# Youncy-Hu/MAGE

Measured on AMD Instinct MI355X. Metric: generated frames/sec (64x64, 16-frame clips), higher is better.
Workload: dtype bf16

## Files before the change

mage_amd/csrc/gemm4.hip:

```cpp
#include <cstdio>
#include <cstdlib>
#include <utility>

#include "gemm_shared.h"
#include "gemm4_regs.h"
#include "attn_mfma.h"

namespace {

struct Gemm4Args {
    const void* A;
    const void* W;
    void* Y;
    const float* bias;
    const float* ln_stats;
    const float* ln_colsum;
    const void* residual;
    float* ln_part;
    void* y2;
    int M, N, K, lda, ldw, ldy, ldr, ldy2, y_dtype, a_off, y_off;
    int ntiles_n, ntiles;
    int stagger_groups, stagger_sleeps;
    alignas(16) int attn_axis;
    float attn_scale;
    int out_w, y_img_stride;
};

#ifndef MAGE4_ABL
#define MAGE4_ABL 0
#endif

#ifdef MAGE4_STAMP
__device__ unsigned long long g4_stamps[256 * 32 * 4 * 8];
#define G4_STAMP(it, p)                                                                                                   \
    do {                                                                                                                  \
        if (lane == 0 && (it) < 32 && blockIdx.x < 256) {                                                                 \
            g4_stamps[((blockIdx.x * 32 + (it)) * 4 + wave) * 8 + (p)] = __builtin_readcyclecounter();                    \
            if ((p) == 1) g4_stamps[((blockIdx.x * 32 + (it)) * 4 + wave) * 8 + 3] = __builtin_amdgcn_s_memrealtime();    \
            if ((p) == 0) g4_stamps[((blockIdx.x * 32 + (it)) * 4 + wave) * 8 + 4] = __builtin_amdgcn_s_memrealtime();    \
        }                                                                                                                 \
    } while (0)
#else
#define G4_STAMP(it, p)
#endif

constexpr int G4_STAGE = 65536, G4_WOFF = 32768, G4_RING = 2 * G4_STAGE, G4_LDS = G4_RING + 4 * 4096;

#ifdef MAGE4_MFMA32
template <int B, bool ZERO, bool CLOB>
__device__ __forceinline__ void g4_mfma32(const u32x4& w, const u32x4& x) {
    if constexpr (ZERO && CLOB) asm volatile("v_mfma_f32_32x32x16_bf16 a[%c2:%c3], %0, %1, 0" ::"v"(w), "v"(x), "i"(16 * B), "i"(16 * B + 15) : G4_ALL_ACC);
    else if constexpr (ZERO) asm volatile("v_mfma_f32_32x32x16_bf16 a[%c2:%c3], %0, %1, 0" ::"v"(w), "v"(x), "i"(16 * B), "i"(16 * B + 15));
    else if constexpr (CLOB) asm volatile("v_mfma_f32_32x32x16_bf16 a[%c2:%c3], %0, %1, a[%c2:%c3]" ::"v"(w), "v"(x), "i"(16 * B), "i"(16 * B + 15) : G4_ALL_ACC);
    else asm volatile("v_mfma_f32_32x32x16_bf16 a[%c2:%c3], %0, %1, a[%c2:%c3]" ::"v"(w), "v"(x), "i"(16 * B), "i"(16 * B + 15));
}
#endif
typedef unsigned g4_u32x2 __attribute__((ext_vector_type(2)));
template <bool HF>
__device__ __forceinline__ f32x4 g4_epi_qk(const u32x4& k, const u32x4& q) {
    f32x4 d;
    if constexpr (HF) asm volatile("s_nop 1\n\tv_mfma_f32_16x16x32_f16 %0, %1, %2, 0\n\ts_nop 15" : "=&v"(d) : "v"(k), "v"(q));
    else asm volatile("s_nop 1\n\tv_mfma_f32_16x16x32_bf16 %0, %1, %2, 0\n\ts_nop 15" : "=&v"(d) : "v"(k), "v"(q));
    return d;
}
#define G4_EPI_PV(OP)                                                                                                                               \
    asm volatile("s_nop 1\n\t" OP " %0, %2, %4, 0\n\t" OP " %1, %3, %4, 0\n\t" OP " %0, %2, %5, %0\n\t" OP " %1, %3, %5, %1\n\ts_nop 15"           \
                 : "=&v"(o0), "=&v"(o1)                                                                                                             \
                 : "v"(__builtin_bit_cast(g4_u32x2, vt0)), "v"(__builtin_bit_cast(g4_u32x2, vt1)), "v"(__builtin_bit_cast(g4_u32x2, phi)),          \
                   "v"(__builtin_bit_cast(g4_u32x2, plo)))
template <bool HF>
__device__ __forceinline__ void g4_epi_pv(const ashort4& vt0, const ashort4& vt1, const ashort4& phi, const ashort4& plo, f32x4& o0, f32x4& o1) {
    if constexpr (HF) G4_EPI_PV("v_mfma_f32_16x16x16_f16");
    else G4_EPI_PV("v_mfma_f32_16x16x16_bf16");
}

template <bool SWAP, int I, bool ZERO, bool CLOB, bool HF>
__device__ __forceinline__ void g4_mm(const u32x4& w, const u32x4& x) {
    if constexpr (SWAP) g4_mfma<I, ZERO, CLOB, HF>(x, w);
    else g4_mfma<I, ZERO, CLOB, HF>(w, x);
}
template <int ACT, int EK, int LN, bool RB, bool HF, bool QF, bool TX = false>
__device__ __forceinline__ void gemm4_body(const Gemm4Args& g) {
    static_assert(EK != EK_GENERAL, "lean epilogue kinds");
    static_assert(!TX || QF, "the temporal row map belongs to the fused attention entry");
    static_assert(!QF || (LN == LN_CONSUME && ACT == MAGE_ACT_NONE), "fused attention: the LayerNorm-consuming in_proj");
    static_assert(!HF || (LN != LN_DUAL && LN != LN_GELUBWD), "f16 form: the generation path's epilogues");
    typedef std::conditional_t<HF, f16_t, unsigned short> H16;
    extern __shared__ __attribute__((aligned(16))) char smem[];
    g4_claim_accumulators();
    const int tid = threadIdx.x;
    const int lane = tid & 63;
    const int wave = __builtin_amdgcn_readfirstlane(tid >> 6);
    const int nwg8 = gridDim.x >> 3;
    const int xcd = blockIdx.x & 7, li = blockIdx.x >> 3;
    const int q8 = g.ntiles >> 3, r8 = g.ntiles & 7;
    const int chunk0 = xcd < r8 ? xcd * (q8 + 1) : r8 * (q8 + 1) + (xcd - r8) * q8;
    const int chunk1 = chunk0 + q8 + (xcd < r8 ? 1 : 0);
    const int nk = g.K >> 6;
    int c_tile = chunk0 + li;
    if (c_tile >= chunk1) return;
    const int last_tile = c_tile + ((chunk1 - 1 - c_tile) / nwg8) * nwg8;

    const int lr = lane >> 3, lp = lane & 7;
    unsigned voffA[8], voffW[8];
    [[maybe_unused]] auto frame_row = [&](int R) {
        if constexpr (TX) return (R & 15) * g.out_w + (R >> 4);
        else return g.attn_axis == 1 ? ((R & 15) << 4) + (R >> 4) : R;
    };
    [[maybe_unused]] auto tile_row0 = [&](int tm_) {
        const int clip = tm_ / g.y_img_stride;
        return (long)clip * 16 * g.out_w + (tm_ - clip * g.y_img_stride) * 16;
    };
#pragma unroll
    for (int u = 0; u < 8; ++u) {
        const int r = u * 8 + lr;
        const int ch = lp ^ ((r >> 1) & 7);
        if constexpr (TX) voffA[u] = (unsigned)frame_row(wave * 64 + r) * (unsigned)(g.lda * 2) + (unsigned)(ch * 16 + 8192 - u * 1024);
        else voffA[u] = (unsigned)((QF ? frame_row(wave * 64 + r) : r) * g.lda * 2 + ch * 16 + 8192 - u * 1024);
        voffW[u] = (unsigned)(r * g.ldw * 2 + ch * 16 + 8192 - u * 1024);
    }
    auto a_base = [&](int tile) {
        if constexpr (TX) return (const char*)g.A + (tile_row0(tile / g.ntiles_n) + g.a_off) * g.lda * 2 - 4096;
        else return (const char*)g.A + ((long)((tile / g.ntiles_n) * 256 + (QF ? 0 : wave * 64)) + g.a_off) * g.lda * 2 - 4096;
    };
    auto w_base = [&](int tile) { return (const char*)g.W + (long)((tile % g.ntiles_n) * (QF ? 384 : 256) + wave * 64) * g.ldw * 2 - 4096; };
    [[maybe_unused]] auto w_base_v = [&](int tile) { return (const char*)g.W + (long)((tile % g.ntiles_n) * 384 + 256 + wave * 32) * g.ldw * 2 - 4096; };
    const char* a_src = a_base(c_tile);
    const char* w_src = w_base(c_tile);
    const char* a_next = a_src;
    const char* w_next = w_src;
    const unsigned lds0 = (unsigned)(uintptr_t)(__attribute__((address_space(3))) char*)smem + wave * 8192 + 4096;
    auto dma_m0 = [&](unsigned lds_group) __attribute__((always_inline)) {
        asm volatile("s_mov_b32 m0, %0\n\ts_nop 0" ::"s"(lds0 + lds_group) : "memory");
    };
    auto dma_m0w = [&](unsigned stage_off, bool half) __attribute__((always_inline)) { dma_m0(stage_off + G4_WOFF - (half ? wave * 4096 : 0)); };

    const int wm = wave >> 1, wn = wave & 1;
    const int l15 = lane & 15, grp = lane >> 4;
    const int rsw = (l15 >> 1) & 7;
    const int pc[2] = {((grp + 0) ^ rsw) * 16, ((grp + 4) ^ rsw) * 16};
    const int x_off = (wm * 128 + l15) * 128;
    const int w_off = G4_WOFF + (wn * 128 + l15) * 128;
    [[maybe_unused]] const int w_off_v = G4_WOFF + (wn * 64 + l15) * 128;
    u32x4 wf[2][8], xf[2][4];
    auto rd_w1 = [&](int buf, int stage, int t, int nt) __attribute__((always_inline)) {
        wf[buf][nt] = *(const u32x4*)(smem + stage * G4_STAGE + w_off + nt * 2048 + pc[t]);
    };
    [[maybe_unused]] auto rd_wv = [&](int buf, int stage, int t, int nt) __attribute__((always_inline)) {
        wf[buf][nt] = *(const u32x4*)(smem + stage * G4_STAGE + w_off_v + nt * 2048 + pc[t]);
    };
    auto rd_x1 = [&](int buf, int stage, int t, int mt) __attribute__((always_inline)) {
        xf[buf][mt & 3] = *(const u32x4*)(smem + stage * G4_STAGE + x_off + mt * 2048 + pc[t]);
    };

#ifdef MAGE4_MFMA32
    const int l31 = lane & 31, hi5 = lane >> 5;
    const int rsw32 = (l31 >> 1) & 7;
    const int x32_off = (wm * 128 + l31) * 128, w32_off = G4_WOFF + (wn * 128 + l31) * 128;
    u32x4 wq[2][4], xq[2][4];
    auto rd_w32 = [&](int buf, int stage, int ks, int nb) __attribute__((always_inline)) {
        wq[buf][nb] = *(const u32x4*)(smem + stage * G4_STAGE + w32_off + nb * 4096 + (((2 * ks + hi5) ^ rsw32) << 4));
    };
    auto rd_x32 = [&](int buf, int stage, int ks, int mb) __attribute__((always_inline)) {
        xq[buf][mb] = *(const u32x4*)(smem + stage * G4_STAGE + x32_off + mb * 4096 + (((2 * ks + hi5) ^ rsw32) << 4));
    };
#endif
    if (g.stagger_groups > 1) {
        for (int w = (li % g.stagger_groups) * g.stagger_sleeps; w > 0; --w) __builtin_amdgcn_s_sleep(16);
    }
    dma_m0(0);
    g4_for<8>([&](auto u_) { g4_dma<decltype(u_)::value>(voffA[decltype(u_)::value], a_src); });
    dma_m0(G4_WOFF);
    g4_for<8>([&](auto u_) { g4_dma<decltype(u_)::value>(voffW[decltype(u_)::value], w_src); });
    a_src += 128;
    w_src += 128;
    dma_m0(G4_STAGE);
    g4_for<8>([&](auto u_) { g4_dma<decltype(u_)::value>(voffA[decltype(u_)::value], a_src); });
    dma_m0(G4_STAGE + G4_WOFF);
    g4_for<8>([&](auto u_) { g4_dma<decltype(u_)::value>(voffW[decltype(u_)::value], w_src); });
    a_src += 128;
    w_src += 128;
    __builtin_amdgcn_s_waitcnt(0x0F70);
    ring_barrier();
#ifdef MAGE4_MFMA32
#pragma unroll
    for (int b = 0; b < 4; ++b) { rd_w32(0, 0, 0, b); rd_x32(0, 0, 0, b); }
#else
#pragma unroll
    for (int nt = 0; nt < 8; ++nt) rd_w1(0, 0, 0, nt);
#pragma unroll
    for (int m = 0; m < 4; ++m) rd_x1(0, 0, 0, m);
#endif

    [[maybe_unused]] int it = 0;
    for (; c_tile < chunk1; c_tile += nwg8, ++it) {
        G4_STAMP(it, 0);
        const int tm = c_tile / g.ntiles_n, tn = c_tile - tm * g.ntiles_n;
        MAGE_DASSERT(c_tile >= 0 && c_tile < g.ntiles && tm * 256 < g.M && tn * (QF ? 384 : 256) < g.N);
        [[maybe_unused]] float ln_mean[8], ln_rstd[8];
        [[maybe_unused]] long row0 = 0;
        if constexpr (TX) row0 = tile_row0(tm);
        auto tile = [&](auto PH_) __attribute__((always_inline)) {
            constexpr int PH = decltype(PH_)::value;
            constexpr bool HALF = PH == 2, KEEP = PH == 1;
            constexpr int NW = HALF ? 4 : 8;
            const int m0 = ((MAGE4_ABL & 32) ? (int)blockIdx.x : tm) * 256 + wm * 128;
            const int n0 = QF ? tn * 384 + (HALF ? 256 + wn * 64 : wn * 128) : ((MAGE4_ABL & 32) ? 0 : tn) * 256 + wn * 128;
            [[maybe_unused]] const int ny0 = HALF ? tn * 128 + wn * 64 : n0;
            if constexpr (KEEP) {
                if constexpr (TX) a_next = (const char*)g.A + (row0 + g.a_off) * g.lda * 2 - 4096;
                else a_next = a_base(c_tile);
                w_next = w_base_v(c_tile);
            } else {
                const int nt_tile = c_tile + nwg8 > last_tile ? last_tile : c_tile + nwg8;
                a_next = a_base(nt_tile);
                w_next = w_base(nt_tile);
            }
            auto rd_w = [&](int buf, int stage, int t, int nt) __attribute__((always_inline)) {
                if constexpr (HALF) rd_wv(buf, stage, t, nt);
                else rd_w1(buf, stage, t, nt);
            };
            f32x4 biasm[2][4];
            [[maybe_unused]] f32x4 lns[2][4];
            [[maybe_unused]] f32x4 pl[4][2];
            [[maybe_unused]] int ql15 = l15, qgrp = grp;
            if constexpr (QF) asm volatile("" : "+v"(ql15), "+v"(qgrp));
            auto slab = [&](auto S_, auto FIRST_, auto LAST_, int j) __attribute__((always_inline)) {
                constexpr int S = decltype(S_)::value;
                constexpr bool FIRST = decltype(FIRST_)::value, LAST = decltype(LAST_)::value;
                constexpr int ACC0 = HALF ? 32 : 0;
                constexpr bool WH_ = LAST ? KEEP : HALF;
                constexpr int WU = WH_ ? 4 : 8;
                g4_for<4 * NW>([&](auto i_) {
                    constexpr int i = decltype(i_)::value, m = i / NW, nt = i % NW;
                    g4_mm<PH == 2, ACC0 + ((nt >> 2) * 8 + m) * 4 + (nt & 3), FIRST, i == 0, HF>(wf[0][nt], xf[0][m]);
                    __builtin_amdgcn_sched_barrier(0);
                    if constexpr (!(MAGE4_ABL & 4) && i < 4) {
                        rd_x1(1, S, 0, 4 + i);
                        __builtin_amdgcn_sched_barrier(0);
                    }
                    if constexpr (!(MAGE4_ABL & 2) && !FIRST && i == 4) {
                        dma_m0w((S ^ 1) * G4_STAGE, WH_);
                        __builtin_amdgcn_sched_barrier(0);
                    }
                    if constexpr (!HALF) {
                        if constexpr (!(MAGE4_ABL & 2) && !FIRST && (i & 3) == 1 && i > 4 && (i >> 2) - 1 < WU) {
                            g4_dma<(i >> 2) - 1>(voffW[(i >> 2) - 1], w_src);
                            __builtin_amdgcn_sched_barrier(0);
                        }
                    } else {
                        if constexpr (!FIRST && i > 4 && i - 5 < WU) {
                            g4_dma<i - 5>(voffW[i - 5], w_src);
                            __builtin_amdgcn_sched_barrier(0);
                        }
                    }
                });
                if constexpr (!(MAGE4_ABL & 2) && !FIRST && !HALF && WU == 8) {
                    g4_dma<7>(voffW[7], w_src);
                    __builtin_amdgcn_sched_barrier(0);
                }
                if constexpr (!(MAGE4_ABL & 8) && !FIRST) w_src = (j == nk - 2) ? w_next : w_src + 128;
                g4_for<4 * NW>([&](auto i_) {
                    constexpr int i = decltype(i_)::value, m = i / NW, nt = i % NW;
                    g4_mm<PH == 2, ACC0 + ((nt >> 2) * 8 + 4 + m) * 4 + (nt & 3), FIRST, i == 0, HF>(wf[0][nt], xf[1][m]);
                    __builtin_amdgcn_sched_barrier(0);
                    if constexpr (!(MAGE4_ABL & 4) && i < 4 + NW) {
                        if constexpr (i < 4) rd_x1(0, S, 1, i);
                        else rd_w(1, S, 1, i - 4);
                        __builtin_amdgcn_sched_barrier(0);
                    }
                });
                if constexpr (LAST) {
#pragma unroll
                    for (int b = 0; b < 4; ++b) {
                        if constexpr (PH == 2) {
                            biasm[0][0][b] = g.bias[n0 + b * 16 + l15];
                            lns[0][0][b] = g.ln_colsum[n0 + b * 16 + l15];
                            continue;
                        }
                        const int n = n0 + b * 16 + grp * 4;
                        biasm[0][b] = *(const f32x4*)(g.bias + n);
                        if constexpr (LN == LN_CONSUME) lns[0][b] = *(const f32x4*)(g.ln_colsum + n);
                    }
                    if constexpr (LN == LN_CONSUME && !HALF) {
#pragma unroll
                        for (int a = 0; a < 8; ++a) {
                            long row;
                            if constexpr (TX) row = row0 + frame_row(wm * 128 + a * 16 + ql15);
                            else row = QF ? (long)tm * 256 + frame_row(wm * 128 + a * 16 + ql15) : (long)(m0 + a * 16 + l15);
                            const float2 st = *(const float2*)(g.ln_stats + 2 * row);
                            ln_mean[a] = st.x;
                            ln_rstd[a] = st.y;
                        }
                    }
                    __builtin_amdgcn_sched_barrier(0);
                }
                g4_for<4 * NW>([&](auto i_) {
                    constexpr int i = decltype(i_)::value, m = i / NW, nt = i % NW;
                    g4_mm<PH == 2, ACC0 + ((nt >> 2) * 8 + m) * 4 + (nt & 3), false, i == 0, HF>(wf[1][nt], xf[0][m]);
                    __builtin_amdgcn_sched_barrier(0);
                    if constexpr (!(MAGE4_ABL & 4) && i < 4) {
                        rd_x1(1, S, 1, 4 + i);
                        __builtin_amdgcn_sched_barrier(0);
                    }
                });
                if constexpr (MAGE4_ABL & 16) __builtin_amdgcn_s_waitcnt(0xC07F);
                else if constexpr (FIRST && QF) __builtin_amdgcn_s_waitcnt(PH == 1 ? 0x007C : 0x0070);
                else if constexpr (FIRST) __builtin_amdgcn_s_waitcnt(LN == LN_CONSUME ? 0x8074 : 0x8070);
                else __builtin_amdgcn_s_waitcnt(0x0070);
                ring_barrier();
                __builtin_amdgcn_sched_barrier(0);
                g4_for<4 * NW>([&](auto i_) {
                    constexpr int i = decltype(i_)::value, m = i / NW, nt = i % NW;
                    g4_mm<PH == 2, ACC0 + ((nt >> 2) * 8 + 4 + m) * 4 + (nt & 3), false, i == 0, HF>(wf[1][nt], xf[1][m]);
                    __builtin_amdgcn_sched_barrier(0);
                    if constexpr (!(MAGE4_ABL & 4) && i < 4 + NW && !LAST) {
                        if constexpr (i < 4) rd_x1(0, S ^ 1, 0, i);
                        else rd_w(0, S ^ 1, 0, i - 4);
                        __builtin_amdgcn_sched_barrier(0);
                    }
                    if constexpr (!(MAGE4_ABL & 2) && !LAST && !HALF) {
                        if constexpr (i == 2) dma_m0(S * G4_STAGE);
                        if constexpr ((i & 3) == 3) g4_dma<(i >> 2)>(voffA[i >> 2], a_src);
                        if constexpr (i == 2 || (i & 3) == 3) __builtin_amdgcn_sched_barrier(0);
                    }
                    if constexpr (!(MAGE4_ABL & 2) && LAST && !HALF) {
                        if constexpr (i == 0) dma_m0(S * G4_STAGE);
                        if constexpr (i == 16) dma_m0w(S * G4_STAGE, WH_);
                        if constexpr ((i & 1) == 1 && i < 16) g4_dma<(i >> 1)>(voffA[i >> 1], a_src);
                        if constexpr ((i & 1) == 1 && i > 16 && ((i - 16) >> 1) < WU) g4_dma<((i - 16) >> 1)>(voffW[(i - 16) >> 1], w_src);
                        if constexpr (i == 0 || i == 16 || (i & 1) == 1) __builtin_amdgcn_sched_barrier(0);
                    }
                    if constexpr (HALF && !LAST) {
                        if constexpr (i == 0) dma_m0(S * G4_STAGE);
                        if constexpr ((i & 1) == 1) g4_dma<(i >> 1)>(voffA[i >> 1], a_src);
                        if constexpr (i == 0 || (i & 1) == 1) __builtin_amdgcn_sched_barrier(0);
                    }
                    if constexpr (HALF && LAST) {
                        if constexpr (i == 0) dma_m0(S * G4_STAGE);
                        if constexpr (i == 8) dma_m0w(S * G4_STAGE, false);
                        if constexpr (i < 8) g4_dma<i>(voffA[i], a_src);
                        else g4_dma<i - 8>(voffW[i - 8], w_src);
                        __builtin_amdgcn_sched_barrier(0);
                    }
                });
                if constexpr (!(MAGE4_ABL & 8)) a_src = (j == nk - 3) ? a_next : a_src + 128;
                if constexpr (!(MAGE4_ABL & 8) && LAST) w_src += 128;
            };
#ifdef MAGE4_MFMA32
            auto slab32 = [&](auto S_, auto FIRST_, auto LAST_, int j) __attribute__((always_inline)) {
                constexpr int S = decltype(S_)::value;
                constexpr bool FIRST = decltype(FIRST_)::value, LAST = decltype(LAST_)::value;
                auto quarter = [&](auto Q_) __attribute__((always_inline)) {
                    constexpr int Q = decltype(Q_)::value, buf = Q & 1;
                    g4_for<16>([&](auto i_) {
                        constexpr int i = decltype(i_)::value, mb = i >> 2, nb = i & 3;
                        g4_mfma32<mb * 4 + nb, FIRST && Q == 0, i == 0>(wq[buf][nb], xq[buf][mb]);
                        __builtin_amdgcn_sched_barrier(0);
                        if constexpr (!(MAGE4_ABL & 4) && i < 8 && !(Q == 3 && LAST)) {
                            constexpr int st = Q == 3 ? (S ^ 1) : S, ks = (Q + 1) & 3;
                            if constexpr (i < 4) rd_x32(buf ^ 1, st, ks, i);
                            else rd_w32(buf ^ 1, st, ks, i - 4);
                            __builtin_amdgcn_sched_barrier(0);
                        }
                        if constexpr (Q == 0 && !(MAGE4_ABL & 2) && !FIRST) {
                            if constexpr (i == 4) dma_m0((S ^ 1) * G4_STAGE + G4_WOFF);
                            if constexpr (i >= 5 && i < 13) g4_dma<i - 5>(voffW[i - 5], w_src);
                            if constexpr (i >= 4 && i < 13) __builtin_amdgcn_sched_barrier(0);
                        }
                        if constexpr (Q == 3 && !(MAGE4_ABL & 2) && !LAST) {
                            if constexpr (i == 1) dma_m0(S * G4_STAGE);
                            if constexpr (i >= 2 && i < 10) g4_dma<i - 2>(voffA[i - 2], a_src);
                            if constexpr (i >= 1 && i < 10) __builtin_amdgcn_sched_barrier(0);
                        }
                    });
                };
                quarter(std::integral_constant<int, 0>{});
                if constexpr (!(MAGE4_ABL & 8) && !FIRST) w_src = (j == nk - 2) ? w_next : w_src + 128;
                quarter(std::integral_constant<int, 1>{});
                quarter(std::integral_constant<int, 2>{});
                if constexpr (FIRST) __builtin_amdgcn_s_waitcnt(0x8070);
                else __builtin_amdgcn_s_waitcnt(0x0070);
                ring_barrier();
                __builtin_amdgcn_sched_barrier(0);
                quarter(std::integral_constant<int, 3>{});
                if constexpr (LAST && !(MAGE4_ABL & 2)) {
                    dma_m0(S * G4_STAGE);
                    g4_for<8>([&](auto u_) { g4_dma<decltype(u_)::value>(voffA[decltype(u_)::value], a_src); });
                    dma_m0(S * G4_STAGE + G4_WOFF);
                    g4_for<8>([&](auto u_) { g4_dma<decltype(u_)::value>(voffW[decltype(u_)::value], w_src); });
                }
                if constexpr (!(MAGE4_ABL & 8)) a_src = (j == nk - 3) ? a_next : a_src + 128;
                if constexpr (!(MAGE4_ABL & 8) && LAST) w_src += 128;
            };
#define slab slab32
#endif
            typedef std::integral_constant<int, 0> S0;
            typedef std::integral_constant<int, 1> S1;
            slab(S0{}, std::true_type{}, std::false_type{}, 0);
            slab(S1{}, std::false_type{}, std::false_type{}, 1);
            for (int j = 2; j < nk - 2; j += 2) {
                slab(S0{}, std::false_type{}, std::false_type{}, j);
                slab(S1{}, std::false_type{}, std::false_type{}, j + 1);
            }
            slab(S0{}, std::false_type{}, std::false_type{}, nk - 2);
            slab(S1{}, std::false_type{}, std::true_type{}, nk - 1);
#ifdef MAGE4_MFMA32
#undef slab
#endif
            asm volatile("s_nop 15\n\ts_nop 7" ::: "memory");
            G4_STAMP(it, 1);
#if MAGE4_ABL & 1
            {
                f32x4 t = g4_acc_read<0>() + g4_acc_read<17>() + g4_acc_read<63>();
                if (t[0] + t[1] + t[2] + t[3] == 123456.789f) ((float*)g.Y)[0] = t[0] + biasm[0][0][0];
            }
#else
            char* win = smem + G4_RING + wave * 4096;
#pragma unroll
            for (int b = 0; b < (HALF ? 0 : 4); ++b) {
                if constexpr (PH == 2) {
                    biasm[1][0][b] = g.bias[n0 + 64 + b * 16 + l15];
                    lns[1][0][b] = g.ln_colsum[n0 + 64 + b * 16 + l15];
                    continue;
                }
                const int n = n0 + 64 + b * 16 + grp * 4;
                biasm[1][b] = *(const f32x4*)(g.bias + n);
                if constexpr (LN == LN_CONSUME) lns[1][b] = *(const f32x4*)(g.ln_colsum + n);
            }
            if constexpr (QF) {
                g4_for<(HALF ? 2 : 4)>([&](auto c_) {
                    constexpr int c = decltype(c_)::value, h = HALF ? 0 : c >> 1, mh = c & 1, ha = HALF ? 1 : h;
                    __builtin_amdgcn_sched_barrier(0);
                    f32x4 t[4][4];
                    g4_for<16>([&](auto q_) {
                        constexpr int q = decltype(q_)::value;
                        t[q >> 2][q & 3] = g4_acc_read<(ha * 8 + mh * 4 + (q >> 2)) * 4 + (q & 3), q == 0>();
                    });
                    if constexpr (PH == 1) {
#pragma unroll
                        for (int mt = 0; mt < 4; ++mt) {
                            uint2 pk[4];
#pragma unroll
                            for (int nt = 0; nt < 4; ++nt) {
                                const f32x4 v = (t[mt][nt] - lns[h][nt] * ln_mean[mh * 4 + mt]) * ln_rstd[mh * 4 + mt] + biasm[h][nt];
                                pk[nt] = uint2{pack16x2<H16>(v[0], v[1]), pack16x2<H16>(v[2], v[3])};
                            }
                            f32x4 st = g4_epi_qk<HF>(u32x4{pk[2].x, pk[2].y, pk[3].x, pk[3].y}, u32x4{pk[0].x, pk[0].y, pk[1].x, pk[1].y});
                            f32x4 p;
                            {
#pragma clang fp contract(off)
                                float mx = -INFINITY;
#pragma unroll
                                for (int e = 0; e < 4; ++e) {
                                    if constexpr (TX) st[e] = (4 * qgrp + e <= ql15) ? st[e] * g.attn_scale : -INFINITY;
                                    else st[e] = st[e] * g.attn_scale;
                                    mx = fmaxf(mx, st[e]);
                                }
                                mx = fmaxf(mx, __shfl_xor(mx, 16));
                                mx = fmaxf(mx, __shfl_xor(mx, 32));
#pragma unroll
                                for (int e = 0; e < 4; ++e) {
                                    if constexpr (TX) p[e] = (4 * qgrp + e <= ql15) ? expf(st[e] - mx) : 0.f;
                                    else p[e] = expf(st[e] - mx);
                                }
                            }
                            pl[mt][0] = p;
                        }
                        g4_for<4>([&](auto mt_) { g4_acc_write<c * 4 + decltype(mt_)::value>(pl[decltype(mt_)::value][0]); });
                    } else {
                        long shift;
                        if constexpr (TX) shift = g.y_off;
                        else shift = (long)(tm * 256 / g.out_w) * (g.y_img_stride - g.out_w) + g.y_off;
                        const int srow = (qgrp * 16 + ql15) >> 3, scc = ql15 & 7;
                        H16* op = (H16*)g.Y + ny0 + h * 64 + scc * 8;
                        const int wchunk = (qgrp & 1) * 2 + (qgrp >> 1);
                        g4_for<8>([&](auto q_) {
                            constexpr int q = decltype(q_)::value, hd = q >> 2, mt = q & 3;
                            pl[mt][hd] = g4_acc_read<(hd * 2 + mh) * 4 + mt>();
                        });
#pragma unroll
                        for (int mt = 0; mt < 4; ++mt) {
                            f32x4 mean4, rstd4;
#pragma unroll
                            for (int e = 0; e < 4; ++e) {
                                mean4[e] = __shfl(ln_mean[mh * 4 + mt], 4 * grp + e);
                                rstd4[e] = __shfl(ln_rstd[mh * 4 + mt], 4 * grp + e);
                            }
#pragma unroll
                            for (int hd = 0; hd < 2; ++hd) {
                                const f32x4 p = pl[mt][hd];
                                float den = 0.f;
                                ashort4 phi, plo;
#pragma unroll
                                for (int e = 0; e < 4; ++e) {
                                    den += p[e];
                                    short ph, pw;
                                    attn_p_split<H16>(p[e], ph, pw);
                                    phi[e] = ph;
                                    plo[e] = pw;
                                }
                                den += __shfl_xor(den, 16);
                                den += __shfl_xor(den, 32);
                                f32x4 o[2];
                                ashort4 vt[2];
#pragma unroll
                                for (int b = 0; b < 2; ++b) {
                                    const int nt = hd * 2 + b;
                                    const f32x4 v = (t[mt][nt] - mean4 * lns[h][0][nt]) * rstd4 + biasm[h][0][nt];
                                    vt[b] = __builtin_bit_cast(ashort4, uint2{pack16x2<H16>(v[0], v[1]), pack16x2<H16>(v[2], v[3])});
                                }
                                g4_epi_pv<HF>(vt[0], vt[1], phi, plo, o[0], o[1]);
                                const float inv = 1.0f / den;
                                f32x4 v0, v1;
#pragma unroll
                                for (int e = 0; e < 4; ++e) {
                                    const auto sw = __builtin_amdgcn_permlane16_swap(__float_as_uint(o[0][e]), __float_as_uint(o[1][e]), false, false);
                                    v0[e] = __uint_as_float(sw[0]) * inv;
                                    v1[e] = __uint_as_float(sw[1]) * inv;
                                }
                                *(u32x4*)(win + ql15 * 128 + (((hd * 4 + wchunk) ^ ((ql15 >> 1) & 7)) << 4)) =
                                    u32x4{pack16x2<H16>(v0[0], v0[1]), pack16x2<H16>(v0[2], v0[3]), pack16x2<H16>(v1[0], v1[1]), pack16x2<H16>(v1[2], v1[3])};
                            }
#pragma unroll
                            for (int i = 0; i < 2; ++i) {
                                const int r = srow + 8 * i;
                                long yrow;
                                if constexpr (TX) yrow = row0 + frame_row(wm * 128 + mh * 64 + mt * 16 + r) + shift;
                                else yrow = (long)tm * 256 + frame_row(wm * 128 + mh * 64 + mt * 16 + r) + shift;
                                *(u32x4*)(op + yrow * g.ldy) = *(const u32x4*)(win + r * 128 + ((scc ^ ((r >> 1) & 7)) << 4));
                            }
                        }
                    }
                });
            } else {
            mage_gemm_desc e = {};
            e.M = 0x7fffffff;
            e.N = LN == LN_PRODUCE ? g.N : 0x7fffffff;
            e.K = g.K;
            e.Y = g.Y;
            e.ldy = g.ldy;
            e.y_dtype = g.y_dtype;
            e.out_h = 1;
            e.out_w = 0x7fffffff;
            e.y_mul_x = 1;
            e.y_off = g.y_off;
            e.y2 = g.y2;
            e.ldy2 = g.ldy2;
            e.ln_part = g.ln_part;
            g4_for<4>([&](auto c_) {
                constexpr int c = decltype(c_)::value, h = c >> 1, mh = c & 1;
                __builtin_amdgcn_sched_barrier(0);
                f32x4 t[4][4];
                g4_for<16>([&](auto q_) {
                    constexpr int q = decltype(q_)::value;
                    t[q >> 2][q & 3] = g4_acc_read<(h * 8 + mh * 4 + (q >> 2)) * 4 + (q & 3), q == 0>();
                });
                [[maybe_unused]] LnConsume lnc;
                if constexpr (LN == LN_CONSUME) {
#pragma unroll
                    for (int a = 0; a < 4; ++a) {
                        lnc.mean[a] = ln_mean[mh * 4 + a];
                        lnc.rstd[a] = ln_rstd[mh * 4 + a];
                    }
#pragma unroll
                    for (int b = 0; b < 4; ++b) lnc.s[b] = lns[h][b];
                    if (g.y_dtype == MAGE_F32) epilogue_lean<ACT, float, 4, false, LN>(e, biasm[h], t, m0 + mh * 64, n0 + h * 64, lane, 1, win, 0, &lnc);
                    else epilogue_lean<ACT, H16, 4, false, LN>(e, biasm[h], t, m0 + mh * 64, n0 + h * 64, lane, 1, win, 0, &lnc);
                } else if constexpr (LN == LN_DUAL || LN == LN_GELUBWD) {
                    epilogue_lean<ACT, unsigned short, 4, false, LN>(e, biasm[h], t, m0 + mh * 64, n0 + h * 64, lane, 1, win, 0);
                } else {
                    if (g.y_dtype == MAGE_F32) epilogue_lean<ACT, float, 4, false, LN>(e, biasm[h], t, m0 + mh * 64, n0 + h * 64, lane, 1, win, 0);
                    else epilogue_lean<ACT, H16, 4, false, LN>(e, biasm[h], t, m0 + mh * 64, n0 + h * 64, lane, 1, win, 0);
                }
            });
            }
#endif
            G4_STAMP(it, 2);
            __builtin_amdgcn_sched_barrier(0);
            if constexpr (KEEP) {
#pragma unroll
                for (int nt = 0; nt < 4; ++nt) rd_wv(0, 0, 0, nt);
#pragma unroll
                for (int m = 0; m < 4; ++m) rd_x1(0, 0, 0, m);
            } else if (c_tile + nwg8 < chunk1) {
#ifdef MAGE4_MFMA32
#pragma unroll
                for (int b = 0; b < 4; ++b) { rd_w32(0, 0, 0, b); rd_x32(0, 0, 0, b); }
#else
#pragma unroll
                for (int nt = 0; nt < 8; ++nt) rd_w1(0, 0, 0, nt);
#pragma unroll
                for (int m = 0; m < 4; ++m) rd_x1(0, 0, 0, m);
#endif
            }
        };
        if constexpr (QF) {
            tile(std::integral_constant<int, 1>{});
            tile(std::integral_constant<int, 2>{});
        } else {
            tile(std::integral_constant<int, 0>{});
        }
    }
}

template <int ACT, int EK, int LN, bool RB, bool HF = false>
__global__ __launch_bounds__(256) void gemm4_kernel(const Gemm4Args g) {
    gemm4_body<ACT, EK, LN, RB, HF, false>(g);
}
template <bool HF>
__global__ __launch_bounds__(256) void gemm4_attn_kernel(const Gemm4Args g) {
    gemm4_body<MAGE_ACT_NONE, EK_BIAS, LN_CONSUME, false, HF, true>(g);
}
template <bool HF>
__global__ __launch_bounds__(256) void gemm4_tattn_kernel(const Gemm4Args g) {
    gemm4_body<MAGE_ACT_NONE, EK_BIAS, LN_CONSUME, false, HF, true, true>(g);
}

template <int ACT, int EK, int LN, bool RB, bool HF = false, bool QF = false, bool TX = false>
int launch4(const mage_gemm_desc* d, hipStream_t s, int n_cu, int attn_axis = 0, float attn_scale = 0.f) {
    Gemm4Args a;
    a.attn_axis = attn_axis;
    a.attn_scale = attn_scale;
    a.out_w = d->out_w;
    a.y_img_stride = d->y_img_stride;
    if constexpr (TX) a.y_img_stride = d->out_w / 16;
    a.A = d->A;
    a.W = d->W;
    a.Y = d->Y;
    a.bias = d->bias ? d->bias : (const float*)mage_zero_page();
    a.ln_stats = d->ln_stats;
    a.ln_colsum = d->ln_colsum;
    a.residual = d->residual;
    a.ln_part = d->ln_part;
    a.y2 = d->y2;
    a.M = d->M;
    a.N = d->N;
    a.K = d->K;
    a.lda = d->lda;
    a.ldw = d->ldw ? d->ldw : d->K;
    a.ldy = d->ldy;
    a.ldr = d->ldr;
    a.ldy2 = d->ldy2;
    a.y_dtype = d->y_dtype;
    a.a_off = d->a_off;
    a.y_off = d->y_off;
    a.ntiles_n = d->N / (QF ? 384 : 256);
    a.ntiles = (d->M / 256) * a.ntiles_n;
    const int st_groups = mage_options().gemm4_stagger_groups, st_percent = mage_options().gemm4_stagger_percent;
    a.stagger_groups = 0;
    a.stagger_sleeps = 0;
    const int grid = a.ntiles >= n_cu ? n_cu : ((a.ntiles + 7) & ~7);
    if (st_groups > 1 && a.ntiles / grid >= 6) {
        const long period = (long)(d->K / 64) * 3100 + 9000;
        a.stagger_groups = st_groups;
        a.stagger_sleeps = (int)(period * st_percent / 100 / st_groups / 1024);
    }
    int r;
    if constexpr (TX) r = mage_gemm_launch<gemm4_tattn_kernel<HF>>(grid, 256, G4_LDS, s, a);
    else if constexpr (QF) r = mage_gemm_launch<gemm4_attn_kernel<HF>>(grid, 256, G4_LDS, s, a);
    else r = mage_gemm_launch<gemm4_kernel<ACT, EK, LN, RB, HF>>(grid, 256, G4_LDS, s, a);
    return r < 0 ? r : 1;
}

}

namespace {

struct Tn4Args {
    const unsigned short* A;
    const unsigned short* B;
    float* P;
    float* DB;
    long lda, ldb, T, tps;
    int N, K, n_split, ntk;
};
typedef short g4_tr4 __attribute__((ext_vector_type(4)));
__device__ __forceinline__ g4_tr4 g4_lds_tr(const char* p) { return __builtin_amdgcn_ds_read_tr16_b64_v4i16((__attribute__((address_space(3))) g4_tr4*)p); }

template <bool DB>
__global__ __launch_bounds__(256) void gemm_tn4_kernel(const Tn4Args g) {
    constexpr int PART = 32768, STAGE = 2 * PART;
    extern __shared__ __attribute__((aligned(16))) char smem[];
    g4_claim_accumulators();
    const int lane = threadIdx.x & 63;
    const int wave = __builtin_amdgcn_readfirstlane(threadIdx.x >> 6);
    const int tile = blockIdx.x / g.n_split, s = blockIdx.x - tile * g.n_split;
    const int tm = tile / g.ntk, tk = tile - tm * g.ntk;
    const long t_begin = (long)s * g.tps;
    const long t_end = t_begin + g.tps < g.T ? t_begin + g.tps : g.T;
    const int nslab = (int)((t_end - t_begin) >> 6);
    const int rr = lane >> 3, pc = lane & 7;
    unsigned voffA[8], voffB[8];
#pragma unroll
    for (int u = 0; u < 8; ++u) {
        const int col_in_strip = (((pc >> 1) ^ (rr & 3) ^ (u & 1)) << 4) + ((pc & 1) << 3);
        voffA[u] = (unsigned)(((long)(u * 8 + rr) * g.lda + wave * 64 + col_in_strip) * 2 + 8192 - u * 1024);
        voffB[u] = (unsigned)(((long)(u * 8 + rr) * g.ldb + wave * 64 + col_in_strip) * 2 + 8192 - u * 1024);
    }
    const char* a_src = (const char*)(g.A + t_begin * g.lda + (long)tm * 256) - 4096;
    const char* b_src = (const char*)(g.B + t_begin * g.ldb + (long)tk * 256) - 4096;
    const long da = 64 * g.lda * 2, db_ = 64 * g.ldb * 2;
    int a_slab = 0, b_slab = 0;
    const unsigned lds0 = (unsigned)(uintptr_t)(__attribute__((address_space(3))) char*)smem + wave * 8192 + 4096;
    auto dma_m0 = [&](unsigned lds_group) __attribute__((always_inline)) {
        asm volatile("s_mov_b32 m0, %0\n\ts_nop 0" ::"s"(lds0 + lds_group) : "memory");
    };
    auto a_advance = [&]() __attribute__((always_inline)) {
        const bool more = a_slab + 1 < nslab;
        a_src = more ? a_src + da : a_src;
        a_slab = more ? a_slab + 1 : a_slab;
    };
    auto b_advance = [&]() __attribute__((always_inline)) {
        const bool more = b_slab + 1 < nslab;
        b_src = more ? b_src + db_ : b_src;
        b_slab = more ? b_slab + 1 : b_slab;
    };
    const int wm = wave >> 1, wn = wave & 1;
    const int i15 = lane & 15, grp = lane >> 4;
    const int lane_off = grp * 1024 + (i15 >> 2) * 128 + (i15 & 3) * 8;
    const int sw = (i15 >> 2) ^ (grp & 1);
    g4_tr4 bfh[2][8][2], afh[2][4][2];
    auto rd_b = [&](int buf, int stage, int t, int nt, int h) __attribute__((always_inline)) {
        bfh[buf][nt][h] = g4_lds_tr(smem + stage * STAGE + PART + ((wn * 2 + (nt >> 2)) * 8 + t * 4) * 1024 + lane_off + (((nt & 3) ^ sw) << 5) + h * 512);
    };
    auto rd_a = [&](int buf, int stage, int t, int mt, int h) __attribute__((always_inline)) {
        afh[buf][mt & 3][h] = g4_lds_tr(smem + stage * STAGE + ((wm * 2 + (mt >> 2)) * 8 + t * 4) * 1024 + lane_off + (((mt & 3) ^ sw) << 5) + h * 512);
    };
    auto frag = [](const g4_tr4 (&h)[2]) __attribute__((always_inline)) {
        return __builtin_bit_cast(u32x4, __builtin_shufflevector(h[0], h[1], 0, 1, 2, 3, 4, 5, 6, 7));
    };
    typedef __attribute__((ext_vector_type(2))) __bf16 bf16x2v;
    const bf16x2v ones2 = {(__bf16)1.0f, (__bf16)1.0f};
    [[maybe_unused]] float dbs[8] = {0.f, 0.f, 0.f, 0.f, 0.f, 0.f, 0.f, 0.f};
    [[maybe_unused]] auto db_acc = [&](int mt, const g4_tr4 (&h)[2]) __attribute__((always_inline)) {
        const uint2 w0 = __builtin_bit_cast(uint2, h[0]), w1 = __builtin_bit_cast(uint2, h[1]);
        float d = dbs[mt];
        d = __builtin_amdgcn_fdot2_f32_bf16(__builtin_bit_cast(bf16x2v, w0.x), ones2, d, false);
        d = __builtin_amdgcn_fdot2_f32_bf16(__builtin_bit_cast(bf16x2v, w0.y), ones2, d, false);
        d = __builtin_amdgcn_fdot2_f32_bf16(__builtin_bit_cast(bf16x2v, w1.x), ones2, d, false);
        d = __builtin_amdgcn_fdot2_f32_bf16(__builtin_bit_cast(bf16x2v, w1.y), ones2, d, false);
        dbs[mt] = d;
    };

    dma_m0(0);
    g4_for<8>([&](auto u_) { g4_dma<decltype(u_)::value>(voffA[decltype(u_)::value], a_src); });
    dma_m0(PART);
    g4_for<8>([&](auto u_) { g4_dma<decltype(u_)::value>(voffB[decltype(u_)::value], b_src); });
    a_advance();
    b_advance();
    dma_m0(STAGE);
    g4_for<8>([&](auto u_) { g4_dma<decltype(u_)::value>(voffA[decltype(u_)::value], a_src); });
    dma_m0(STAGE + PART);
    g4_for<8>([&](auto u_) { g4_dma<decltype(u_)::value>(voffB[decltype(u_)::value], b_src); });
    a_advance();
    b_advance();
    __builtin_amdgcn_s_waitcnt(0x0F70);
    ring_barrier();
#pragma unroll
    for (int nt = 0; nt < 8; ++nt) { rd_b(0, 0, 0, nt, 0); rd_b(0, 0, 0, nt, 1); }
#pragma unroll
    for (int m = 0; m < 4; ++m) { rd_a(0, 0, 0, m, 0); rd_a(0, 0, 0, m, 1); }

    auto slab = [&](auto S_, auto FIRST_) __attribute__((always_inline)) {
        constexpr int S = decltype(S_)::value;
        constexpr bool FIRST = decltype(FIRST_)::value;
        g4_for<32>([&](auto i_) {
            constexpr int i = decltype(i_)::value, m = i >> 3, nt = i & 7;
            g4_mfma<m * 8 + nt, FIRST, i == 0>(frag(bfh[0][nt]), frag(afh[0][m]));
            __builtin_amdgcn_sched_barrier(0);
            if constexpr (i < 8) {
                rd_a(1, S, 0, 4 + (i >> 1), i & 1);
                __builtin_amdgcn_sched_barrier(0);
            }
            if constexpr (DB && nt == 7) {
                db_acc(m, afh[0][m]);
                __builtin_amdgcn_sched_barrier(0);
            }
            if constexpr (!FIRST && i == 8) {
                dma_m0((S ^ 1) * STAGE + PART);
                __builtin_amdgcn_sched_barrier(0);
            }
            if constexpr (!FIRST && i > 8 && (i & 1) == 1 && i < 25) {
                g4_dma<((i - 9) >> 1)>(voffB[(i - 9) >> 1], b_src);
                __builtin_amdgcn_sched_barrier(0);
            }
        });
        if constexpr (!FIRST) b_advance();
        g4_for<32>([&](auto i_) {
            constexpr int i = decltype(i_)::value, m = i >> 3, nt = i & 7;
            g4_mfma<(4 + m) * 8 + nt, FIRST, i == 0>(frag(bfh[0][nt]), frag(afh[1][m]));
            __builtin_amdgcn_sched_barrier(0);
            if constexpr (i < 24) {
                if constexpr (i < 8) rd_a(0, S, 1, i >> 1, i & 1);
                else rd_b(1, S, 1, (i - 8) >> 1, i & 1);
                __builtin_amdgcn_sched_barrier(0);
            }
            if constexpr (DB && nt == 7) {
                db_acc(4 + m, afh[1][m]);
                __builtin_amdgcn_sched_barrier(0);
            }
        });
        g4_for<32>([&](auto i_) {
            constexpr int i = decltype(i_)::value, m = i >> 3, nt = i & 7;
            g4_mfma<m * 8 + nt, false, i == 0>(frag(bfh[1][nt]), frag(afh[0][m]));
            __builtin_amdgcn_sched_barrier(0);
            if constexpr (i < 8) {
                rd_a(1, S, 1, 4 + (i >> 1), i & 1);
                __builtin_amdgcn_sched_barrier(0);
            }
            if constexpr (DB && nt == 7) {
                db_acc(m, afh[0][m]);
                __builtin_amdgcn_sched_barrier(0);
            }
        });
        __builtin_amdgcn_s_waitcnt(0x0070);
        ring_barrier();
        __builtin_amdgcn_sched_barrier(0);
        g4_for<32>([&](auto i_) {
            constexpr int i = decltype(i_)::value, m = i >> 3, nt = i & 7;
            g4_mfma<(4 + m) * 8 + nt, false, i == 0>(frag(bfh[1][nt]), frag(afh[1][m]));
            __builtin_amdgcn_sched_barrier(0);
            if constexpr (i < 24) {
                if constexpr (i < 8) rd_a(0, S ^ 1, 0, i >> 1, i & 1);
                else rd_b(0, S ^ 1, 0, (i - 8) >> 1, i & 1);
                __builtin_amdgcn_sched_barrier(0);
            }
            if constexpr (DB && nt == 7) {
                db_acc(4 + m, afh[1][m]);
                __builtin_amdgcn_sched_barrier(0);
            }
            if constexpr (i == 24) {
                dma_m0(S * STAGE);
                __builtin_amdgcn_sched_barrier(0);
            }
        });
        g4_for<8>([&](auto u_) { g4_dma<decltype(u_)::value>(voffA[decltype(u_)::value], a_src); });
        __builtin_amdgcn_sched_barrier(0);
        a_advance();
    };
    typedef std::integral_constant<int, 0> S0;
    typedef std::integral_constant<int, 1> S1;
    slab(S0{}, std::true_type{});
    int j = 1;
    for (; j + 1 < nslab; j += 2) {
        slab(S1{}, std::false_type{});
        slab(S0{}, std::false_type{});
    }
    if (j < nslab) slab(S1{}, std::false_type{});
    asm volatile("s_nop 15\n\ts_nop 7" ::: "memory");
    float* out = g.P + ((long)s * g.N + (long)tm * 256 + wm * 128) * g.K + (long)tk * 256 + wn * 128;
    g4_for<64>([&](auto q_) {
        constexpr int q = decltype(q_)::value, mt = q >> 3, nt = q & 7;
        *(f32x4*)(out + (long)(mt * 16 + i15) * g.K + nt * 16 + grp * 4) = g4_acc_read<q, (q & 15) == 0>();
    });
    if constexpr (DB) {
#pragma unroll
        for (int mt = 0; mt < 8; ++mt) {
            float v = dbs[mt];
            v += __shfl_xor(v, 16);
            v += __shfl_xor(v, 32);
            if (grp == 0) g.DB[(long)s * g.N + (long)tm * 256 + wm * 128 + mt * 16 + i15] = v;
        }
    }
}

}

int mage_gemm4h_try(const mage_gemm_desc* d, hipStream_t s, int n_cu);

int mage_gemm4_try(const mage_gemm_desc* d, hipStream_t s) {
    const bool hf = d->dtype == MAGE_F16;
    if ((d->dtype != MAGE_BF16 && !hf) || d->n_split > 1) return 0;
    if (mage_options().gemm_no_4w) return 0;
    if (d->M % 256 || d->N % 256 || d->K % 128 || d->K < 256 || d->K > 1024) return 0;
    if (d->taps_h * d->taps_w != 1 || d->stride != 1 || d->dy0 || d->dx0 || d->in_h != d->out_h || d->in_w != d->out_w || d->a_half) return 0;
    if (d->out_h != 1 || d->out_w < d->M || d->y_mul_x != 1) return 0;
    if (d->scale || d->rowadd || d->post_relu || d->res_half) return 0;
    if (d->residual || d->ln_part || d->rowadd) return 0;
    if (!d->bias && (d->N > 4096 || d->ln_stats || mage_zero_page() == nullptr)) return 0;
    if ((d->ln_colsum != nullptr) != (d->ln_stats != nullptr)) return 0;
// ... 124 lines not shown
```

Measured before the change: 6561.

## Batch fused-attention epilogue MFMAs and software-pipeline output stores

In the fused QKV/attention epilogue of the persistent GEMM, the four QK MFMAs are now issued in one asm block, and so are the PV MFMAs for both head halves. This replaces the per-tile blocks that each paid a trailing s_nop 15 wait. Row reductions use permlane16/32 swaps instead of shfl_xor. The output address is hoisted out of the loop, and each tile's global stores are deferred to overlap with the next tile's MFMAs using a double-buffered LDS half. Optional stamp instrumentation for the attention phases is also added. The batching raises register pressure, and the deferred stores depend on the two LDS halves not aliasing.

```diff
diff --git a/mage_amd/csrc/gemm4.hip b/mage_amd/csrc/gemm4.hip
--- a/mage_amd/csrc/gemm4.hip
+++ b/mage_amd/csrc/gemm4.hip
@@ -40,8 +40,15 @@
             if ((p) == 0) g4_stamps[((blockIdx.x * 32 + (it)) * 4 + wave) * 8 + 4] = __builtin_amdgcn_s_memrealtime();    \
         }                                                                                                                 \
     } while (0)
+__device__ unsigned g4_qstamps[256 * 32 * 4 * 10];
+#define G4_QSTAMP(k)                                                  \
+    do {                                                              \
+        qst[(k)] = (unsigned)__builtin_readcyclecounter();            \
+        qst[5 + (k)] = (unsigned)__builtin_amdgcn_s_memrealtime();    \
+    } while (0)
 #else
 #define G4_STAMP(it, p)
+#define G4_QSTAMP(k)
 #endif
 
 constexpr int G4_STAGE = 65536, G4_WOFF = 32768, G4_RING = 2 * G4_STAGE, G4_LDS = G4_RING + 4 * 4096;
@@ -56,22 +63,51 @@
 }
 #endif
 typedef unsigned g4_u32x2 __attribute__((ext_vector_type(2)));
+#define G4_EPI_QK4(OP)                                                                                                                              \
+    asm volatile("s_nop 1\n\t" OP " %0, %4, %5, 0\n\t" OP " %1, %6, %7, 0\n\t" OP " %2, %8, %9, 0\n\t" OP " %3, %10, %11, 0\n\ts_nop 15"             \
+                 : "=&v"(d[0]), "=&v"(d[1]), "=&v"(d[2]), "=&v"(d[3])                                                                               \
+                 : "v"(k[0]), "v"(q[0]), "v"(k[1]), "v"(q[1]), "v"(k[2]), "v"(q[2]), "v"(k[3]), "v"(q[3]))
 template <bool HF>
-__device__ __forceinline__ f32x4 g4_epi_qk(const u32x4& k, const u32x4& q) {
-    f32x4 d;
-    if constexpr (HF) asm volatile("s_nop 1\n\tv_mfma_f32_16x16x32_f16 %0, %1, %2, 0\n\ts_nop 15" : "=&v"(d) : "v"(k), "v"(q));
-    else asm volatile("s_nop 1\n\tv_mfma_f32_16x16x32_bf16 %0, %1, %2, 0\n\ts_nop 15" : "=&v"(d) : "v"(k), "v"(q));
-    return d;
-}
-#define G4_EPI_PV(OP)                                                                                                                               \
-    asm volatile("s_nop 1\n\t" OP " %0, %2, %4, 0\n\t" OP " %1, %3, %4, 0\n\t" OP " %0, %2, %5, %0\n\t" OP " %1, %3, %5, %1\n\ts_nop 15"           \
-                 : "=&v"(o0), "=&v"(o1)                                                                                                             \
-                 : "v"(__builtin_bit_cast(g4_u32x2, vt0)), "v"(__builtin_bit_cast(g4_u32x2, vt1)), "v"(__builtin_bit_cast(g4_u32x2, phi)),          \
-                   "v"(__builtin_bit_cast(g4_u32x2, plo)))
+__device__ __forceinline__ void g4_epi_qk4(const u32x4 (&k)[4], const u32x4 (&q)[4], f32x4 (&d)[4]) {
+    if constexpr (HF) G4_EPI_QK4("v_mfma_f32_16x16x32_f16");
+    else G4_EPI_QK4("v_mfma_f32_16x16x32_bf16");
+}
+#define G4_EPI_PV2(OP)                                                                                                                              \
+    asm volatile("s_nop 1\n\t" OP " %0, %4, %8, 0\n\t" OP " %1, %5, %8, 0\n\t" OP " %2, %6, %10, 0\n\t" OP " %3, %7, %10, 0\n\t"                    \
+                 OP " %0, %4, %9, %0\n\t" OP " %1, %5, %9, %1\n\t" OP " %2, %6, %11, %2\n\t" OP " %3, %7, %11, %3\n\ts_nop 15"                        \
+                 : "=&v"(o[0][0]), "=&v"(o[0][1]), "=&v"(o[1][0]), "=&v"(o[1][1])                                                                   \
+                 : "v"(__builtin_bit_cast(g4_u32x2, vt[0][0])), "v"(__builtin_bit_cast(g4_u32x2, vt[0][1])),                                       \
+                   "v"(__builtin_bit_cast(g4_u32x2, vt[1][0])), "v"(__builtin_bit_cast(g4_u32x2, vt[1][1])),                                       \
+                   "v"(__builtin_bit_cast(g4_u32x2, phi[0])), "v"(__builtin_bit_cast(g4_u32x2, plo[0])),                                           \
+                   "v"(__builtin_bit_cast(g4_u32x2, phi[1])), "v"(__builtin_bit_cast(g4_u32x2, plo[1])))
 template <bool HF>
-__device__ __forceinline__ void g4_epi_pv(const ashort4& vt0, const ashort4& vt1, const ashort4& phi, const ashort4& plo, f32x4& o0, f32x4& o1) {
-    if constexpr (HF) G4_EPI_PV("v_mfma_f32_16x16x16_f16");
-    else G4_EPI_PV("v_mfma_f32_16x16x16_bf16");
+__device__ __forceinline__ void g4_epi_pv2(const ashort4 (&vt)[2][2], const ashort4 (&phi)[2], const ashort4 (&plo)[2], f32x4 (&o)[2][2]) {
+    if constexpr (HF) G4_EPI_PV2("v_mfma_f32_16x16x16_f16");
+    else G4_EPI_PV2("v_mfma_f32_16x16x16_bf16");
+}
+__device__ __forceinline__ void g4_xchg16(float v, float& a, float& b) {
+    const auto r = __builtin_amdgcn_permlane16_swap(__float_as_uint(v), __float_as_uint(v), false, false);
+    a = __uint_as_float(r[0]);
+    b = __uint_as_float(r[1]);
+}
+__device__ __forceinline__ void g4_xchg32(float v, float& a, float& b) {
+    const auto r = __builtin_amdgcn_permlane32_swap(__float_as_uint(v), __float_as_uint(v), false, false);
+    a = __uint_as_float(r[0]);
+    b = __uint_as_float(r[1]);
+}
+__device__ __forceinline__ float g4_max4(float v) {
+    float a, b;
+    g4_xchg16(v, a, b);
+    v = fmaxf(a, b);
+    g4_xchg32(v, a, b);
+    return fmaxf(a, b);
+}
+__device__ __forceinline__ float g4_sum4(float v) {
+    float a, b;
+    g4_xchg16(v, a, b);
+    v = a + b;
+    g4_xchg32(v, a, b);
+    return a + b;
 }
 
 template <bool SWAP, int I, bool ZERO, bool CLOB, bool HF>
@@ -193,8 +229,11 @@
 #endif
 
     [[maybe_unused]] int it = 0;
+#ifdef MAGE4_STAMP
+    [[maybe_unused]] unsigned qst[10];
+#endif
     for (; c_tile < chunk1; c_tile += nwg8, ++it) {
-        G4_STAMP(it, 0);
+        if constexpr (QF) { G4_QSTAMP(0); } else { G4_STAMP(it, 0); }
         const int tm = c_tile / g.ntiles_n, tn = c_tile - tm * g.ntiles_n;
         MAGE_DASSERT(c_tile >= 0 && c_tile < g.ntiles && tm * 256 < g.M && tn * (QF ? 384 : 256) < g.N);
         [[maybe_unused]] float ln_mean[8], ln_rstd[8];
@@ -409,7 +448,7 @@
 #undef slab
 #endif
             asm volatile("s_nop 15\n\ts_nop 7" ::: "memory");
-            G4_STAMP(it, 1);
+            if constexpr (QF) { G4_QSTAMP(PH == 1 ? 1 : 3); } else { G4_STAMP(it, 1); }
 #if MAGE4_ABL & 1
             {
                 f32x4 t = g4_acc_read<0>() + g4_acc_read<17>() + g4_acc_read<63>();
@@ -429,6 +468,26 @@
                 if constexpr (LN == LN_CONSUME) lns[1][b] = *(const f32x4*)(g.ln_colsum + n);
             }
             if constexpr (QF) {
+                [[maybe_unused]] char* ybase = nullptr;
+                [[maybe_unused]] long ystep_seq = 0, ystep_r8 = 0;
+                if constexpr (HALF) {
+                    long shift;
+                    if constexpr (TX) shift = g.y_off;
+                    else shift = (long)(tm * 256 / g.out_w) * (g.y_img_stride - g.out_w) + g.y_off;
+                    const int srow0 = (qgrp * 16 + ql15) >> 3;
+                    long yrow0;
+                    if constexpr (TX) yrow0 = row0 + frame_row(wm * 128 + srow0) + shift;
+                    else yrow0 = (long)tm * 256 + frame_row(wm * 128 + srow0) + shift;
+                    ybase = (char*)((H16*)g.Y + ny0 + (ql15 & 7) * 8 + yrow0 * g.ldy);
+                    const long rowb = (long)g.ldy * (long)sizeof(H16);
+                    if constexpr (TX) {
+                        ystep_seq = rowb;
+                        ystep_r8 = 8 * (long)g.out_w * rowb;
+                    } else {
+                        ystep_seq = g.attn_axis == 1 ? rowb : 16 * rowb;
+                        ystep_r8 = g.attn_axis == 1 ? 128 * rowb : 8 * rowb;
+                    }
+                }
                 g4_for<(HALF ? 2 : 4)>([&](auto c_) {
                     constexpr int c = decltype(c_)::value, h = HALF ? 0 : c >> 1, mh = c & 1, ha = HALF ? 1 : h;
                     __builtin_amdgcn_sched_barrier(0);
@@ -438,6 +497,7 @@
                         t[q >> 2][q & 3] = g4_acc_read<(ha * 8 + mh * 4 + (q >> 2)) * 4 + (q & 3), q == 0>();
                     });
                     if constexpr (PH == 1) {
+                        u32x4 kf[4], qf[4];
 #pragma unroll
                         for (int mt = 0; mt < 4; ++mt) {
                             uint2 pk[4];
@@ -446,7 +506,14 @@
                                 const f32x4 v = (t[mt][nt] - lns[h][nt] * ln_mean[mh * 4 + mt]) * ln_rstd[mh * 4 + mt] + biasm[h][nt];
                                 pk[nt] = uint2{pack16x2<H16>(v[0], v[1]), pack16x2<H16>(v[2], v[3])};
                             }
-                            f32x4 st = g4_epi_qk<HF>(u32x4{pk[2].x, pk[2].y, pk[3].x, pk[3].y}, u32x4{pk[0].x, pk[0].y, pk[1].x, pk[1].y});
+                            kf[mt] = u32x4{pk[2].x, pk[2].y, pk[3].x, pk[3].y};
+                            qf[mt] = u32x4{pk[0].x, pk[0].y, pk[1].x, pk[1].y};
+                        }
+                        f32x4 st4[4];
+                        g4_epi_qk4<HF>(kf, qf, st4);
+#pragma unroll
+                        for (int mt = 0; mt < 4; ++mt) {
+                            f32x4 st = st4[mt];
                             f32x4 p;
                             {
 #pragma clang fp contract(off)
@@ -457,8 +524,7 @@
                                     else st[e] = st[e] * g.attn_scale;
                                     mx = fmaxf(mx, st[e]);
                                 }
-                                mx = fmaxf(mx, __shfl_xor(mx, 16));
-                                mx = fmaxf(mx, __shfl_xor(mx, 32));
+                                mx = g4_max4(mx);
 #pragma unroll
                                 for (int e = 0; e < 4; ++e) {
                                     if constexpr (TX) p[e] = (4 * qgrp + e <= ql15) ? expf(st[e] - mx) : 0.f;
@@ -469,68 +535,74 @@
                         }
                         g4_for<4>([&](auto mt_) { g4_acc_write<c * 4 + decltype(mt_)::value>(pl[decltype(mt_)::value][0]); });
                     } else {
-                        long shift;
-                        if constexpr (TX) shift = g.y_off;
-                        else shift = (long)(tm * 256 / g.out_w) * (g.y_img_stride - g.out_w) + g.y_off;
                         const int srow = (qgrp * 16 + ql15) >> 3, scc = ql15 & 7;
-                        H16* op = (H16*)g.Y + ny0 + h * 64 + scc * 8;
                         const int wchunk = (qgrp & 1) * 2 + (qgrp >> 1);
                         g4_for<8>([&](auto q_) {
                             constexpr int q = decltype(q_)::value, hd = q >> 2, mt = q & 3;
                             pl[mt][hd] = g4_acc_read<(hd * 2 + mh) * 4 + mt>();
                         });
+                        f32x4 mean4[4], rstd4[4];
 #pragma unroll
                         for (int mt = 0; mt < 4; ++mt) {
-                            f32x4 mean4, rstd4;
 #pragma unroll
                             for (int e = 0; e < 4; ++e) {
-                                mean4[e] = __shfl(ln_mean[mh * 4 + mt], 4 * grp + e);
-                                rstd4[e] = __shfl(ln_rstd[mh * 4 + mt], 4 * grp + e);
+                                mean4[mt][e] = __shfl(ln_mean[mh * 4 + mt], 4 * grp + e);
+                                rstd4[mt][e] = __shfl(ln_rstd[mh * 4 + mt], 4 * grp + e);
                             }
+                        }
+                        u32x4 rows[2];
+                        auto store_rows = [&](int mt) __attribute__((always_inline)) {
+#pragma unroll
+                            for (int i = 0; i < 2; ++i) *(u32x4*)(ybase + (mh * 4 + mt) * ystep_seq + i * ystep_r8) = rows[i];
+                        };
+#pragma unroll
+                        for (int mt = 0; mt < 4; ++mt) {
+                            char* const whalf = win + (mt & 1) * 2048;
+                            f32x4 o[2][2];
+                            ashort4 vt[2][2], phi[2], plo[2];
+                            float den[2];
 #pragma unroll
                             for (int hd = 0; hd < 2; ++hd) {
                                 const f32x4 p = pl[mt][hd];
-                                float den = 0.f;
-                                ashort4 phi, plo;
+                                den[hd] = 0.f;
 #pragma unroll
                                 for (int e = 0; e < 4; ++e) {
-                                    den += p[e];
+                                    den[hd] += p[e];
                                     short ph, pw;
                                     attn_p_split<H16>(p[e], ph, pw);
-                                    phi[e] = ph;
-                                    plo[e] = pw;
+                                    phi[hd][e] = ph;
+                                    plo[hd][e] = pw;
                                 }
-                                den += __shfl_xor(den, 16);
-                                den += __shfl_xor(den, 32);
-                                f32x4 o[2];
-                                ashort4 vt[2];
+                                den[hd] = g4_sum4(den[hd]);
 #pragma unroll
                                 for (int b = 0; b < 2; ++b) {
                                     const int nt = hd * 2 + b;
-                                    const f32x4 v = (t[mt][nt] - mean4 * lns[h][0][nt]) * rstd4 + biasm[h][0][nt];
-                                    vt[b] = __builtin_bit_cast(ashort4, uint2{pack16x2<H16>(v[0], v[1]), pack16x2<H16>(v[2], v[3])});
+                                    const f32x4 v = (t[mt][nt] - mean4[mt] * lns[h][0][nt]) * rstd4[mt] + biasm[h][0][nt];
+                                    vt[hd][b] = __builtin_bit_cast(ashort4, uint2{pack16x2<H16>(v[0], v[1]), pack16x2<H16>(v[2], v[3])});
                                 }
-                                g4_epi_pv<HF>(vt[0], vt[1], phi, plo, o[0], o[1]);
-                                const float inv = 1.0f / den;
+                            }
+                            g4_epi_pv2<HF>(vt, phi, plo, o);
+                            if (mt > 0) store_rows(mt - 1);
+#pragma unroll
+                            for (int hd = 0; hd < 2; ++hd) {
+                                const float inv = 1.0f / den[hd];
                                 f32x4 v0, v1;
 #pragma unroll
                                 for (int e = 0; e < 4; ++e) {
-                                    const auto sw = __builtin_amdgcn_permlane16_swap(__float_as_uint(o[0][e]), __float_as_uint(o[1][e]), false, false);
+                                    const auto sw = __builtin_amdgcn_permlane16_swap(__float_as_uint(o[hd][0][e]), __float_as_uint(o[hd][1][e]), false, false);
                                     v0[e] = __uint_as_float(sw[0]) * inv;
                                     v1[e] = __uint_as_float(sw[1]) * inv;
                                 }
-                                *(u32x4*)(win + ql15 * 128 + (((hd * 4 + wchunk) ^ ((ql15 >> 1) & 7)) << 4)) =
+                                *(u32x4*)(whalf + ql15 * 128 + (((hd * 4 + wchunk) ^ ((ql15 >> 1) & 7)) << 4)) =
                                     u32x4{pack16x2<H16>(v0[0], v0[1]), pack16x2<H16>(v0[2], v0[3]), pack16x2<H16>(v1[0], v1[1]), pack16x2<H16>(v1[2], v1[3])};
                             }
 #pragma unroll
                             for (int i = 0; i < 2; ++i) {
                                 const int r = srow + 8 * i;
-                                long yrow;
-                                if constexpr (TX) yrow = row0 + frame_row(wm * 128 + mh * 64 + mt * 16 + r) + shift;
-                                else yrow = (long)tm * 256 + frame_row(wm * 128 + mh * 64 + mt * 16 + r) + shift;
-                                *(u32x4*)(op + yrow * g.ldy) = *(const u32x4*)(win + r * 128 + ((scc ^ ((r >> 1) & 7)) << 4));
+                                rows[i] = *(const u32x4*)(whalf + r * 128 + ((scc ^ ((r >> 1) & 7)) << 4));
                             }
                         }
+                        store_rows(3);
                     }
                 });
             } else {
@@ -576,7 +648,15 @@
             });
             }
 #endif
-            G4_STAMP(it, 2);
+            if constexpr (QF) { G4_QSTAMP(PH == 1 ? 2 : 4); } else { G4_STAMP(it, 2); }
+#ifdef MAGE4_STAMP
+            if constexpr (PH == 2) {
+                unsigned v = qst[0];
+#pragma unroll
+                for (int k = 1; k < 10; ++k) v = lane == k ? qst[k] : v;
+                if (lane < 10 && it < 32 && blockIdx.x < 256) g4_qstamps[((blockIdx.x * 32 + it) * 4 + wave) * 10 + lane] = v;
+            }
+#endif
             __builtin_amdgcn_sched_barrier(0);
             if constexpr (KEEP) {
 #pragma unroll
```

Result: no change. 6610, median of 6 (+0.7%).
